# 5l1v3r1/PBS

Measured on AMD Instinct MI355X. Metric: co-run slowdown (%) vs solo + aggregate throughput, 4-tenant mix at 1/2/4/8 GPU, higher is better.
Workload: dtype bf16

## Files before the change

csrc/hip/common.hpp:

```cpp
#pragma once
#include <hip/hip_runtime.h>

#include <cstdint>
#include <cstdio>
#include <cstdlib>

namespace gpbs_hip {

constexpr int kXcds = 8;
constexpr int kMaxTenants = 64;
constexpr int kNumPmc = 4;
constexpr uint32_t kNoOwner = 0xFFFFFFFFu;
constexpr uint32_t kSplitBit = 0x80000000u;
constexpr uint32_t kOwnerMask = 0x7FFFFFFFu;

typedef __bf16 bf16x8 __attribute__((ext_vector_type(8)));
typedef float f32x4 __attribute__((ext_vector_type(4)));
typedef float f32x16 __attribute__((ext_vector_type(16)));
typedef unsigned int u32x4 __attribute__((ext_vector_type(4)));
typedef unsigned int u32x2 __attribute__((ext_vector_type(2)));
typedef unsigned short u16;
typedef unsigned int u32;
typedef unsigned long long u64;

constexpr int kCtx = 4;
struct alignas(64) PartTable {
  u32 epoch;
  u32 flags;
  u32 hold;
  u32 pad0;
  union {
    u32 owner[kXcds * kCtx];
    u64 pair[kXcds][2];
  };
  u32 pad[12];
};
static_assert(sizeof(PartTable) == 192, "partition table layout");

struct alignas(64) WorkQueue {
  u32 next;
  u32 done;
  u32 exited;
  u32 stopped;
  u32 xnext[kXcds];
  u32 pad[4];
};

__device__ __forceinline__ void finish(WorkQueue* q, u32* status, u32 total) {
  if (threadIdx.x == 0) {
    asm volatile("s_waitcnt vmcnt(0)" ::: "memory");
    const u32 old = atomicAdd(&q->exited, 1u);
    if (old == gridDim.x - 1) {
      const u32 d = __hip_atomic_load(&q->done, __ATOMIC_RELAXED, __HIP_MEMORY_SCOPE_AGENT);
      if (status) __hip_atomic_store(status, d | 0x80000000u, __ATOMIC_RELAXED, __HIP_MEMORY_SCOPE_SYSTEM);
      __hip_atomic_store(&q->exited, 0u, __ATOMIC_RELAXED, __HIP_MEMORY_SCOPE_AGENT);
      __hip_atomic_store(&q->stopped, 0u, __ATOMIC_RELAXED, __HIP_MEMORY_SCOPE_AGENT);
      if (d >= total) {
        __hip_atomic_store(&q->next, 0u, __ATOMIC_RELAXED, __HIP_MEMORY_SCOPE_AGENT);
        __hip_atomic_store(&q->done, 0u, __ATOMIC_RELAXED, __HIP_MEMORY_SCOPE_AGENT);
#pragma unroll
        for (int x = 0; x < kXcds; ++x) __hip_atomic_store(&q->xnext[x], 0u, __ATOMIC_RELAXED, __HIP_MEMORY_SCOPE_AGENT);
      }
    }
  }
}


enum GateMode : u32 {
  GATE_NONE = 0, GATE_TABLE = 1, GATE_PARK = 2, GATE_DEVTABLE = 4, GATE_SPATIAL = 8,
  GATE_WAVEPRIO = 16,
  GATE_SE = 32,
  GATE_HOLD = 64,
};
constexpr u32 kParkSpins = 100;
constexpr u32 kHoldSpins = 256;

#define HIPCHECK(x)                                                                              \
  do {                                                                                           \
    hipError_t _e = (x);                                                                         \
    if (_e != hipSuccess) {                                                                      \
      fprintf(stderr, "[gpbs-hip] %s:%d %s -> %s\n", __FILE__, __LINE__, #x, hipGetErrorString(_e)); \
      return -(int)_e - 1000;                                                                    \
    }                                                                                            \
  } while (0)

__device__ __forceinline__ u32 xcc_id() {
  return __builtin_amdgcn_s_getreg((3 << 11) | (0 << 6) | 20);
}

__device__ __forceinline__ u32 hw_id() { return __builtin_amdgcn_s_getreg((31 << 11) | (0 << 6) | 4); }

__device__ __forceinline__ u32 cu_half() { return (hw_id() >> 14) & 1u; }

__device__ __forceinline__ u32 se_id() { return (hw_id() >> 13) & 3u; }

__device__ __forceinline__ u32 load_sys(const u32* p) {
  return __hip_atomic_load(p, __ATOMIC_RELAXED, __HIP_MEMORY_SCOPE_SYSTEM);
}

__device__ __forceinline__ void hold_wait(const PartTable* t, u32 mode) {
  if (!(mode & GATE_HOLD)) return;
  for (u32 k = 0; k < kHoldSpins; ++k) {
    const u32 h = (mode & GATE_DEVTABLE) ? __hip_atomic_load(&t->hold, __ATOMIC_RELAXED, __HIP_MEMORY_SCOPE_AGENT)
                                         : __hip_atomic_load(&t->hold, __ATOMIC_RELAXED, __HIP_MEMORY_SCOPE_SYSTEM);
    if (!h) return;
    __builtin_amdgcn_s_sleep(32);
  }
}

__device__ __forceinline__ bool owns(const PartTable* t, u32 mode, u32 me, u32 xcc) {
  if ((mode & 3) == GATE_NONE) return true;
  if (mode & GATE_SE) {
    const u32 se = se_id();
    const u32* w = t->owner + kCtx * (xcc & 7) + se;
    const u32 o = (mode & GATE_DEVTABLE) ? __hip_atomic_load(w, __ATOMIC_RELAXED, __HIP_MEMORY_SCOPE_AGENT)
                                         : __hip_atomic_load(w, __ATOMIC_RELAXED, __HIP_MEMORY_SCOPE_SYSTEM);
    return (o & kOwnerMask) == me;
  }
  const u64* q = t->pair[xcc & 7];
  const u64 p01 = (mode & GATE_DEVTABLE) ? __hip_atomic_load(q, __ATOMIC_RELAXED, __HIP_MEMORY_SCOPE_AGENT)
                                         : __hip_atomic_load(q, __ATOMIC_RELAXED, __HIP_MEMORY_SCOPE_SYSTEM);
  const u32 w0 = (u32)p01, w1 = (u32)(p01 >> 32);
  const bool h0 = (w0 & kOwnerMask) == me, h1 = (w1 & kOwnerMask) == me;
  if (!(mode & GATE_SPATIAL) || (h0 && h1)) {
    if (h0 || h1) return true;
    const u64 p23 = (mode & GATE_DEVTABLE) ? __hip_atomic_load(q + 1, __ATOMIC_RELAXED, __HIP_MEMORY_SCOPE_AGENT)
                                           : __hip_atomic_load(q + 1, __ATOMIC_RELAXED, __HIP_MEMORY_SCOPE_SYSTEM);
    return (u32)p23 == me || (u32)(p23 >> 32) == me;
  }
  if (h0) return !(w0 & kSplitBit) || cu_half() == 0;
  if (h1) return !(w1 & kSplitBit) || cu_half() == 1;
  return false;
}

__device__ __forceinline__ void count(u64* cnt, u32 me, u32 xcc, u64 inst, u64 cyc, u64 refs, u64 miss) {
  if (!cnt) return;
  u64* c = cnt + ((size_t)me * kXcds + (xcc & 7)) * kNumPmc;
  if (inst) __hip_atomic_fetch_add(c + 0, inst, __ATOMIC_RELAXED, __HIP_MEMORY_SCOPE_SYSTEM);
  if (cyc) __hip_atomic_fetch_add(c + 1, cyc, __ATOMIC_RELAXED, __HIP_MEMORY_SCOPE_SYSTEM);
  if (refs) __hip_atomic_fetch_add(c + 2, refs, __ATOMIC_RELAXED, __HIP_MEMORY_SCOPE_SYSTEM);
  if (miss) __hip_atomic_fetch_add(c + 3, miss, __ATOMIC_RELAXED, __HIP_MEMORY_SCOPE_SYSTEM);
}

__device__ __forceinline__ int grab_unit(WorkQueue* q, const PartTable* table, u32 mode, u32 me, u32 xcc,
                                         int* s_slot, u32 total) {
  if (threadIdx.x == 0) {
    int u = -1;
    hold_wait(table, mode);
    for (u32 spins = 0;; ++spins) {
      if (owns(table, mode, me, xcc)) {
        const u32 t = atomicAdd(&q->next, 1u);
        u = t < total ? (int)t : -1;
        break;
      }
      if ((mode & 3) != GATE_PARK || spins >= kParkSpins ||
          __hip_atomic_load(&q->next, __ATOMIC_RELAXED, __HIP_MEMORY_SCOPE_AGENT) >= total) {
        atomicAdd(&q->stopped, 1u);
        break;
      }
#pragma unroll
      for (int k = 0; k < 6; ++k) __builtin_amdgcn_s_sleep(127);
    }
    *s_slot = u;
  }
  __syncthreads();
  int u = *s_slot;
  __syncthreads();
  return u;
}


__device__ __forceinline__ void count_unit(u64* cnt, u32 me, u32 xcc, u64 inst, u64* t_last, u64 refs, u64 miss,
                                           WorkQueue* q) {
  if (threadIdx.x != 0) return;
  const u64 t = __builtin_amdgcn_s_memtime();
  count(cnt, me, xcc, inst, t - *t_last, refs, miss);
  *t_last = t;
  atomicAdd(&q->done, 1u);
}

}
```

csrc/hip/tenant_kernels.hip:

```cpp
#include "common.hpp"

namespace gpbs_hip {


__device__ __forceinline__ int grab_unit_x(WorkQueue* q, const PartTable* table, u32 mode, u32 me, u32 xcc,
                                           int* s_slot, u32 total) {
  if (threadIdx.x == 0) {
    int u = -1;
    hold_wait(table, mode);
    const u32 per = (total + kXcds - 1) / kXcds;
    for (u32 spins = 0;; ++spins) {
      if (owns(table, mode, me, xcc)) {
        for (u32 k = 0; k < (u32)kXcds; ++k) {
          const u32 r = (xcc + k) & (kXcds - 1);
          const u32 lo = r * per, hi = min(lo + per, total);
          if (lo >= hi) continue;
          if (__hip_atomic_load(&q->xnext[r], __ATOMIC_RELAXED, __HIP_MEMORY_SCOPE_AGENT) >= hi - lo) continue;
          const u32 t = atomicAdd(&q->xnext[r], 1u);
          if (t < hi - lo) {
            u = (int)(lo + t);
            atomicAdd(&q->next, 1u);
            break;
          }
        }
        break;
      }
      if ((mode & 3) != GATE_PARK || spins >= kParkSpins ||
          __hip_atomic_load(&q->next, __ATOMIC_RELAXED, __HIP_MEMORY_SCOPE_AGENT) >= total) {
        atomicAdd(&q->stopped, 1u);
        break;
      }
#pragma unroll
      for (int k = 0; k < 6; ++k) __builtin_amdgcn_s_sleep(127);
    }
    *s_slot = u;
  }
  __syncthreads();
  int u = *s_slot;
  __syncthreads();
  return u;
}


__device__ __forceinline__ u16 f2bf(float x) { return __builtin_bit_cast(u16, (__bf16)x); }
__device__ __forceinline__ float bf2f(u16 x) { return __uint_as_float(((u32)x) << 16); }

constexpr int GBM = 128, GBN = 128, GBK = 64, GNT = 256;
constexpr int kGemmLds = 2 * 2 * GBM * GBK * 2;

typedef __attribute__((address_space(3))) char lds_t;

__device__ __forceinline__ void glds16(const void* g, lds_t* l) {
  __builtin_amdgcn_global_load_lds(g, (__attribute__((address_space(3))) void*)l, 16, 0, 0);
}

__global__ __launch_bounds__(GNT, 2) void k_gemm_bf16_tn(const u16* __restrict__ A, const u16* __restrict__ Bt,
                                                         u16* __restrict__ C, int M, int N, int K, WorkQueue* q,
                                                         const PartTable* table, u32 mode, u32 me, u64* cnt,
                                                         u32 inst_per_tile, u32 refs_per_tile, u32 miss_per_tile,
                                                         u32* status) {
  __shared__ __attribute__((aligned(16))) char smem[kGemmLds + 16];
  lds_t* lds = (lds_t*)smem;
  int* s_slot = (int*)(smem + kGemmLds);
  const u32 xcc = xcc_id();
  u64 t_last = __builtin_amdgcn_s_memtime();
  const int tid = threadIdx.x, lane = tid & 63, wid = tid >> 6;
  const int wr = wid >> 1, wc = wid & 1;
  const int tiles_m = M / GBM, tiles_n = N / GBN, ntiles = tiles_m * tiles_n;
  const int nk = K / GBK;
  constexpr int GROUP_M = 8;

  int srow[4], scol[4];
#pragma unroll
  for (int j = 0; j < 4; ++j) {
    const int c = wid * 4 + j;
    srow[j] = 8 * c + (lane >> 3);
    scol[j] = (((lane & 7) ^ (srow[j] & 7)) * 8);
  }

  for (;;) {
    const int t = grab_unit(q, table, mode, me, xcc, s_slot, (u32)ntiles);
    if (t < 0) break;
    const int in_group = GROUP_M * tiles_n;
    const int g = t / in_group;
    const int first_m = g * GROUP_M;
    const int gsz = min(tiles_m - first_m, GROUP_M);
    const int tm = first_m + (t % in_group) % gsz;
    const int tn = (t % in_group) / gsz;
    const u16* Ab = A + (size_t)tm * GBM * K;
    const u16* Bb = Bt + (size_t)tn * GBN * K;

    f32x4 acc[4][4];
#pragma unroll
// ... 5 lines not shown
      lds_t* la = lds + buf * (2 * GBM * GBK * 2);
      lds_t* lb = la + GBM * GBK * 2;
#pragma unroll
      for (int j = 0; j < 4; ++j) {
        const int c = wid * 4 + j;
        glds16(Ab + (size_t)srow[j] * K + kt * GBK + scol[j], la + c * 1024);
        glds16(Bb + (size_t)srow[j] * K + kt * GBK + scol[j], lb + c * 1024);
      }
    };

    stage(0, 0);
    asm volatile("s_waitcnt vmcnt(0)" ::: "memory");
    __syncthreads();
    int cur = 0;
    for (int kt = 0; kt < nk; ++kt) {
      if (kt + 1 < nk) stage(cur ^ 1, kt + 1);
      const lds_t* la = lds + cur * (2 * GBM * GBK * 2);
      const lds_t* lb = la + GBM * GBK * 2;
#pragma unroll
      for (int s = 0; s < 2; ++s) {
        bf16x8 a[4], b[4];
        const int chunk = s * 4 + (lane >> 4);
#pragma unroll
        for (int i = 0; i < 4; ++i) {
          const int ra = wr * 64 + i * 16 + (lane & 15);
          a[i] = *(const __attribute__((address_space(3))) bf16x8*)(la + ra * 128 + ((chunk ^ (ra & 7)) << 4));
          const int rb = wc * 64 + i * 16 + (lane & 15);
          b[i] = *(const __attribute__((address_space(3))) bf16x8*)(lb + rb * 128 + ((chunk ^ (rb & 7)) << 4));
        }
#pragma unroll
        for (int i = 0; i < 4; ++i)
#pragma unroll
          for (int j = 0; j < 4; ++j) acc[i][j] = __builtin_amdgcn_mfma_f32_16x16x32_bf16(a[i], b[j], acc[i][j], 0, 0, 0);
      }
      asm volatile("s_waitcnt vmcnt(0)" ::: "memory");
      __syncthreads();
      cur ^= 1;
    }
#pragma unroll
    for (int i = 0; i < 4; ++i)
#pragma unroll
      for (int j = 0; j < 4; ++j) {
        const int m = tm * GBM + wr * 64 + i * 16 + (lane >> 4) * 4;
        const int n = tn * GBN + wc * 64 + j * 16 + (lane & 15);
#pragma unroll
        for (int r = 0; r < 4; ++r) C[(size_t)(m + r) * N + n] = f2bf(acc[i][j][r]);
      }
    count_unit(cnt, me, xcc, inst_per_tile, &t_last, refs_per_tile, miss_per_tile, q);
  }
  finish(q, status, (u32)ntiles);
}

constexpr int G2_BM = 256, G2_BK = 64, G2_NT = 512;
constexpr u32 kGemmXRange = 1u << 16;
constexpr u32 kGemmBlock2D = 1u << 17;
constexpr u32 kGemmStatic = 1u << 18;
constexpr int kGemmOptsLive = 1 | 8 | 1 << 23;
constexpr int kGemmOptsShipped = 256 | 8192 | 65536 | 131072;
static int g_gemm_opts = 8;
constexpr int kG2Half = 128 * 128;
constexpr int kG2Buf = 4 * kG2Half;
constexpr int kG2Lds = 2 * kG2Buf;

__device__ __forceinline__ int g2_swz(int r) { return (r >> 1) & 7; }

__global__ __launch_bounds__(G2_NT, 1) void k_gemm256_bf16_tn(const u16* __restrict__ A, const u16* __restrict__ Bt,
                                                             u16* __restrict__ C, int M, int N, int K, WorkQueue* q,
                                                             const PartTable* table, u32 mode, u32 me, u64* cnt,
                                                             u32 inst_per_tile, u32 refs_per_tile, u32 miss_per_tile,
                                                             u32* status) {
  __shared__ __attribute__((aligned(16))) char smem[kG2Lds + 16];
  lds_t* lds = (lds_t*)smem;
  int* s_slot = (int*)(smem + kG2Lds);
  const u32 xcc = xcc_id();
  u64 t_last = __builtin_amdgcn_s_memtime();
  const int tid = threadIdx.x, lane = tid & 63, wid = tid >> 6;
  const int wu = __builtin_amdgcn_readfirstlane(wid);
  const int wr = wu >> 2, wc = wu & 3;
  const int tiles_m = M / G2_BM, tiles_n = N / G2_BM, ntiles = tiles_m * tiles_n;
  const int nt = K / G2_BK;
  int soff[2];
#pragma unroll
  for (int j = 0; j < 2; ++j) {
    const int row = 8 * (2 * wid + j) + (lane >> 3);
    soff[j] = row * K + (((lane & 7) ^ g2_swz(row)) * 8);
  }
  int soffa[4];
#pragma unroll
  for (int j = 0; j < 4; ++j) {
    const int row = 8 * (4 * (wid & 3) + j) + (lane >> 3);
    soffa[j] = row * K + (((lane & 7) ^ g2_swz(row)) * 8);
  }
  const int l16 = lane & 15, lq = lane >> 4;
  const int bh = wc >> 1, bc = (wc & 1) * 64;
  int units_seen = 0;

  for (;;) {
    const int tile = (mode & kGemmStatic) ? (units_seen ? -1 : (int)blockIdx.x)
                     : (mode & kGemmXRange) ? grab_unit_x(q, table, mode, me, xcc, s_slot, (u32)ntiles)
                                            : grab_unit(q, table, mode, me, xcc, s_slot, (u32)ntiles);
    if (tile < 0) break;
    int tm = tile / tiles_n, tn = tile % tiles_n;
    if ((mode & kGemmBlock2D) && (tiles_m & 3) == 0 && (tiles_n & 1) == 0 && ntiles % kXcds == 0) {
      const int per = ntiles / kXcds;
      const int bm = tiles_m / 4, bn = tiles_n / 2;
      const int g = (mode & kGemmXRange) ? tile / per : tile % kXcds;
      const int jj = (mode & kGemmXRange) ? tile % per : tile / kXcds;
      tm = (g >> 1) * bm + jj / bn;
      tn = (g & 1) * bn + jj % bn;
    }
    const u16* Ab = A + (size_t)tm * G2_BM * K;
    const u16* Bb = Bt + (size_t)tn * G2_BM * K;
    auto stage = [&](int kind, int h, int t) {
      const u16* src = (kind ? Bb : Ab) + (size_t)h * 128 * K + t * G2_BK;
      lds_t* dst = lds + (t & 1) * kG2Buf + (kind * 2 + h) * kG2Half + wid * 2048;
      glds16(src + soff[0], dst);
      glds16(src + soff[1], dst + 1024);
    };
    auto stage_own_a = [&](int t) {
      const u16* src = Ab + (size_t)wr * 128 * K + t * G2_BK;
      lds_t* dst = lds + (t & 1) * kG2Buf + wr * kG2Half + (wid & 3) * 4096;
#pragma unroll
      for (int j = 0; j < 4; ++j) glds16(src + soffa[j], dst + j * 1024);
    };
    auto frag = [&](int b, int kind, int h, int r0, int s) -> bf16x8 {
      const int r = r0 + l16;
      const lds_t* p = lds + b * kG2Buf + (kind * 2 + h) * kG2Half + r * 128 + (((4 * s + lq) ^ g2_swz(r)) << 4);
      return *(const __attribute__((address_space(3))) bf16x8*)p;
    };
    f32x4 acc[8][4];
#pragma unroll
    for (int i = 0; i < 8; ++i)
#pragma unroll
      for (int j = 0; j < 4; ++j) acc[i][j] = f32x4{0.f, 0.f, 0.f, 0.f};
    stage(1, 0, 0); stage(1, 1, 0); stage(0, 0, 0); stage(0, 1, 0);
    asm volatile("s_waitcnt vmcnt(0)" ::: "memory");
    __builtin_amdgcn_s_barrier();
    if (wr == 1) __builtin_amdgcn_s_barrier();
    bf16x8 a[4][2], b[4][2];
    for (int t = 0; t < nt; ++t) {
      const int buf = t & 1;
      const bool more = t + 1 < nt;
#pragma unroll
      for (int j = 0; j < 4; ++j)
#pragma unroll
        for (int s2 = 0; s2 < 2; ++s2) b[j][s2] = frag(buf, 1, bh, bc + j * 16, s2);
      __builtin_amdgcn_sched_barrier(0);
#pragma unroll
      for (int i = 0; i < 4; ++i)
#pragma unroll
        for (int s2 = 0; s2 < 2; ++s2) a[i][s2] = frag(buf, 0, wr, i * 16, s2);
      if (more) {
        stage(1, 0, t + 1); stage(1, 1, t + 1);
      } else {
        asm volatile("s_waitcnt vmcnt(0)" ::: "memory");
      }
      __builtin_amdgcn_s_barrier();
      asm volatile("s_waitcnt lgkmcnt(0)" ::: "memory");
      __builtin_amdgcn_s_setprio(1);
#pragma unroll
      for (int s2 = 0; s2 < 2; ++s2)
#pragma unroll
        for (int i = 0; i < 4; ++i)
// ... 41 lines not shown
      const int row = p * 16 + (tid >> 5), c16 = tid & 31;
      u32x4 v = *(const __attribute__((address_space(3))) u32x4*)(lds + row * 512 + (((2 * c16) ^ (row & 14)) << 3));
      if (row & 1) v = u32x4{v.z, v.w, v.x, v.y};
      u32x4* dst = (u32x4*)(C + (size_t)(tm * G2_BM + row) * N + tn * G2_BM + c16 * 8);
      __builtin_nontemporal_store(v, dst);
    }
    __syncthreads();
    ++units_seen;
    if (!(mode & kGemmStatic)) count_unit(cnt, me, xcc, inst_per_tile, &t_last, refs_per_tile, miss_per_tile, q);
  }
  if (!(mode & kGemmStatic)) finish(q, status, (u32)ntiles);
}

constexpr int SNT = 256, SUNROLL = 16, RUNROLL = 6;

template <int U, bool NTS>
__global__ __launch_bounds__(SNT) void k_stream_copy(const f32x4* __restrict__ src, f32x4* __restrict__ dst,
                                                    u64 n4, u32 chunk4, WorkQueue* q, const PartTable* table, u32 mode,
                                                    u32 me, u64* cnt, u32* status) {
  __shared__ int s_slot[4];
  const u32 xcc = xcc_id();
  u64 t_last = __builtin_amdgcn_s_memtime();
  const u32 nchunks = (u32)((n4 + chunk4 - 1) / chunk4);
  const u64 lines = (u64)chunk4 * 16 / 128;
  const u64 inst = (u64)chunk4 * 2 / 64 + 8;
  for (;;) {
    const int c = grab_unit(q, table, mode, me, xcc, s_slot, nchunks);
    if (c < 0) break;
    const u64 base = (u64)c * chunk4;
    const u64 end = min(base + chunk4, n4);
    for (u64 i = base + threadIdx.x; i < end; i += (u64)SNT * U) {
      f32x4 v[U];
#pragma unroll
      for (int k = 0; k < U; ++k) {
        const u64 idx = i + (u64)k * SNT;
        if (idx < end) v[k] = __builtin_nontemporal_load(src + idx);
      }
#pragma unroll
      for (int k = 0; k < U; ++k) {
        const u64 idx = i + (u64)k * SNT;
        if (idx < end) {
          if constexpr (NTS)
            __builtin_nontemporal_store(v[k], dst + idx);
          else
            dst[idx] = v[k];
        }
      }
    }
    count_unit(cnt, me, xcc, inst, &t_last, 2 * lines, 2 * lines, q);
  }
  finish(q, status, nchunks);
}

template <int NT, int U, bool NTL, bool NTS>
__global__ __launch_bounds__(NT) void k_reduce_bf16(const u32x4* __restrict__ a, const u32x4* __restrict__ b,
                                                    u32x4* __restrict__ out, u64 n8, u32 chunk8, WorkQueue* q,
                                                    const PartTable* table, u32 mode, u32 me, u64* cnt,
                                                    u32* status) {
  __shared__ int s_slot[4];
  const u32 xcc = xcc_id();
  u64 t_last = __builtin_amdgcn_s_memtime();
  const u32 nchunks = (u32)((n8 + chunk8 - 1) / chunk8);
  const u64 lines = (u64)chunk8 * 16 / 128;
  const u64 inst = (u64)chunk8 * 3 / 64 + (u64)chunk8 * 16 / 64;
  for (;;) {
    const int c = grab_unit(q, table, mode, me, xcc, s_slot, nchunks);
    if (c < 0) break;
    const u64 base = (u64)c * chunk8, end = min(base + chunk8, n8);
    for (u64 i = base + threadIdx.x; i < end; i += (u64)NT * U) {
      u32x4 x[U], y[U];
#pragma unroll
      for (int k = 0; k < U; ++k) {
        const u64 idx = i + (u64)k * NT;
        if (idx < end) {
          if constexpr (NTL) {
            x[k] = __builtin_nontemporal_load(a + idx);
            y[k] = __builtin_nontemporal_load(b + idx);
          } else {
            x[k] = a[idx];
            y[k] = b[idx];
          }
        }
      }
#pragma unroll
      for (int k = 0; k < U; ++k) {
        const u64 idx = i + (u64)k * NT;
        if (idx >= end) continue;
        const u32* px = (const u32*)&x[k];
        const u32* py = (const u32*)&y[k];
        u32x4 r;
        u32* pr = (u32*)&r;
#pragma unroll
        for (int w = 0; w < 4; ++w) {
          const float lo = bf2f((u16)(px[w] & 0xffff)) + bf2f((u16)(py[w] & 0xffff));
          const float hi = bf2f((u16)(px[w] >> 16)) + bf2f((u16)(py[w] >> 16));
          pr[w] = (u32)f2bf(lo) | ((u32)f2bf(hi) << 16);
        }
        if constexpr (NTS)
          __builtin_nontemporal_store(r, out + idx);
        else
          out[idx] = r;
      }
    }
    count_unit(cnt, me, xcc, inst, &t_last, 3 * lines, 3 * lines, q);
  }
  finish(q, status, nchunks);
}

// ... 65 lines not shown

__global__ void k_census(u32* out, const PartTable* table, u32 mode, u32 me) {
  const u32 xcc = xcc_id();
  const bool ok = owns(table, mode, me, xcc);
  if (threadIdx.x == 0) {
    out[blockIdx.x * 4 + 0] = xcc;
    out[blockIdx.x * 4 + 1] = hw_id();
    out[blockIdx.x * 4 + 2] = ok ? 1u : 0u;
    out[blockIdx.x * 4 + 3] = 0xC0FFEEu;
  }
  if (ok) {
    u64 t = __builtin_amdgcn_s_memtime();
    while (__builtin_amdgcn_s_memtime() - t < 2000) __builtin_amdgcn_s_sleep(1);
  }
}

}

using namespace gpbs_hip;

extern "C" {

int gpbs_hip_set_gemm_opts(int opts) {
  const int old = g_gemm_opts;
  if (opts < 0) return old;
  const int gone = opts & ~(kGemmOptsLive | kGemmOptsShipped);
  static bool warned = false;
  if (gone && !warned) {
    warned = true;
    fprintf(stderr,
            "gpbs_hip_set_gemm_opts: bits 0x%x select GEMM variants that were removed (docs/gemm_lab.md); "
            "the shipped schedule runs\n",
            gone);
  }
  g_gemm_opts = opts & kGemmOptsLive;
  return old;
}

int gpbs_hip_gemm_units(int M, int N) {
  if (M % G2_BM == 0 && N % G2_BM == 0) return (M / G2_BM) * (N / G2_BM);
  return (M / GBM) * (N / GBN);
}

int gpbs_hip_gemm_bf16(const void* A, const void* Bt, void* C, int M, int N, int K, void* q, const void* table,
                       unsigned mode, unsigned me, void* cnt, void* status, int grid, hipStream_t s) {
  if (M % GBM || N % GBN || K % GBK || M <= 0 || N <= 0 || K <= 0) return -22;
  if (M % G2_BM == 0 && N % G2_BM == 0) {
    const int ntiles = (M / G2_BM) * (N / G2_BM);
    if (grid <= 0) grid = 256;
    if (grid > ntiles) grid = ntiles;
    const u32 inst = (u32)((G2_BM / 16) * (G2_BM / 16) * (K / 32) + (K / G2_BK) * 64 + 128);
    const u32 refs = (u32)(((u64)2 * G2_BM * K * 2) / 128);
    const u32 miss = (u32)((((u64)M + N) * K * 2 / 128) / ntiles + (u64)G2_BM * G2_BM * 2 / 128);
    const u32 m2 = mode | ((g_gemm_opts & 1) ? kGemmXRange : 0u) |
                   ((g_gemm_opts & 8) && ntiles % kXcds == 0 ? kGemmBlock2D : 0u) |
                   ((g_gemm_opts & (1 << 23)) && (mode & 3) == GATE_NONE && grid == ntiles ? kGemmStatic : 0u);
    hipLaunchKernelGGL(k_gemm256_bf16_tn, dim3(grid), dim3(G2_NT), 0, s, (const u16*)A, (const u16*)Bt, (u16*)C, M, N,
                       K, (WorkQueue*)q, (const PartTable*)table, m2, me, (u64*)cnt, inst, refs, miss, (u32*)status);
    return hipGetLastError() == hipSuccess ? 0 : -5;
  }
  const int ntiles = (M / GBM) * (N / GBN);
  if (grid <= 0) grid = 256 * 2;
  if (grid > ntiles) grid = ntiles;
  const u32 inst = (u32)((GBM / 16) * (GBN / 16) * (K / 32) * 2 + (K / GBK) * 32 + 64);
  const u32 refs = (u32)(((u64)(GBM + GBN) * K * 2) / 128);
  const u32 miss = (u32)((((u64)M + N) * K * 2 / 128) / ntiles + (u64)GBM * GBN * 2 / 128);
  hipLaunchKernelGGL(k_gemm_bf16_tn, dim3(grid), dim3(GNT), 0, s, (const u16*)A, (const u16*)Bt, (u16*)C, M, N, K,
                     (WorkQueue*)q, (const PartTable*)table, mode, me, (u64*)cnt, inst, refs, miss, (u32*)status);
  return hipGetLastError() == hipSuccess ? 0 : -5;
}

static int g_stream_opts = 0;

int gpbs_hip_set_stream_opts(int opts) {
  const int old = g_stream_opts;
  if (opts >= 0) g_stream_opts = opts;
  return old;
}

int gpbs_hip_stream_copy(const void* src, void* dst, unsigned long long bytes, unsigned chunk_bytes, void* q,
                         const void* table, unsigned mode, unsigned me, void* cnt, void* status, int grid, hipStream_t s) {
  if (bytes % 16 || chunk_bytes % 16 || chunk_bytes == 0) return -22;
  if (grid <= 0) grid = 256;
  using K = void (*)(const f32x4*, f32x4*, u64, u32, WorkQueue*, const PartTable*, u32, u32, u64*, u32*);
  static const K tab[4] = {k_stream_copy<SUNROLL, true>, k_stream_copy<SUNROLL, false>, k_stream_copy<8, true>,
                           k_stream_copy<8, false>};
  hipLaunchKernelGGL(tab[g_stream_opts & 3], dim3(grid), dim3(SNT), 0, s, (const f32x4*)src, (f32x4*)dst, bytes / 16,
                     chunk_bytes / 16, (WorkQueue*)q, (const PartTable*)table, mode, me, (u64*)cnt, (u32*)status);
  return hipGetLastError() == hipSuccess ? 0 : -5;
}

static int g_reduce_opts = 8;

int gpbs_hip_set_reduce_opts(int opts) {
  const int old = g_reduce_opts;
  if (opts >= 0) g_reduce_opts = opts;
  return old;
}

int gpbs_hip_reduce_bf16(const void* a, const void* b, void* out, unsigned long long bytes, unsigned chunk_bytes,
                         void* q, const void* table, unsigned mode, unsigned me, void* cnt, void* status, int grid, hipStream_t s) {
  if (bytes % 16 || chunk_bytes % 16 || chunk_bytes == 0) return -22;
  if (grid <= 0) grid = 256;
  using K = void (*)(const u32x4*, const u32x4*, u32x4*, u64, u32, WorkQueue*, const PartTable*, u32, u32, u64*, u32*);
#define RV(NT, U) {k_reduce_bf16<NT, U, true, true>, k_reduce_bf16<NT, U, false, true>, \
                   k_reduce_bf16<NT, U, true, false>, k_reduce_bf16<NT, U, false, false>}
  static const K table256[4][4] = {RV(256, 6), RV(256, 8), RV(256, 4), RV(256, 12)};
  static const K table512[4][4] = {RV(512, 6), RV(512, 8), RV(512, 4), RV(512, 12)};
#undef RV
  const int o = g_reduce_opts;
  const int nt = (o & 16) ? 512 : 256;
  const K kern = ((o & 16) ? table512 : table256)[o & 3][((o >> 2) & 1) | (((o >> 3) & 1) << 1)];
  hipLaunchKernelGGL(kern, dim3(grid), dim3(nt), 0, s, (const u32x4*)a, (const u32x4*)b, (u32x4*)out,
                     bytes / 16, chunk_bytes / 16, (WorkQueue*)q, (const PartTable*)table, mode, me, (u64*)cnt, (u32*)status);
  return hipGetLastError() == hipSuccess ? 0 : -5;
}

int gpbs_hip_gemv_bf16(const void* W, const void* x, void* y, int R, int K, void* q, const void* table, unsigned mode,
                       unsigned me, void* cnt, void* status, int grid, hipStream_t s) {
  if (K % 512 || R <= 0) return -22;
  if (grid <= 0) grid = (R + 15) / 16;
  if (grid > 256) grid = 256;
  hipLaunchKernelGGL(k_gemv_bf16, dim3(grid), dim3(256), 0, s, (const u16*)W, (const u16*)x, (float*)y, R, K,
                     (WorkQueue*)q, (const PartTable*)table, mode, me, (u64*)cnt, (u32*)status);
  return hipGetLastError() == hipSuccess ? 0 : -5;
}

int gpbs_hip_census(void* out, int blocks, const void* table, unsigned mode, unsigned me, hipStream_t s) {
  hipLaunchKernelGGL(k_census, dim3(blocks), dim3(64), 0, s, (u32*)out, (const PartTable*)table, mode, me);
  return hipGetLastError() == hipSuccess ? 0 : -5;
}

}
```

csrc/hip/runtime.cpp:

```cpp
#include <hip/hip_runtime.h>
#include <hsa/hsa.h>
#include <hsa/hsa_ext_amd.h>
#include <rocprofiler-sdk-roctx/roctx.h>
#include <x86intrin.h>

#include <algorithm>
#include <atomic>
#include <cmath>
#include <cstdio>
#include <cstdlib>
#include <chrono>
#include <condition_variable>
#include <cstring>
#include <deque>
#include <memory>
#include <mutex>
#include <thread>
#include <vector>

#include "../include/gpbs/gpbs.h"
#include "common.hpp"
#include "hwc_attr.h"

using namespace gpbs_hip;
// ... 1414 lines not shown
        hipEventDestroy(retired_ev[i]);
        retired_ev[i] = retired_ev.back();
        retired_ev.pop_back();
      } else {
        ++i;
      }
    hipEvent_t e = nullptr;
    if (hipEventCreateWithFlags(&e, hipEventDisableTiming) != hipSuccess) {
      hipStreamSynchronize(s);
      return;
    }
    hipEventRecord(e, s);
    retired_ev.push_back(e);
  }
  void drain_retired() {
    for (hipEvent_t e : retired_ev) {
      hipEventSynchronize(e);
      hipEventDestroy(e);
    }
    retired_ev.clear();
  }
  uint32_t key_bits = 0;
  int key_half = -1;
  double key_load = 0;
  int64_t rate_t0 = 0;
  uint64_t rate_l0 = 0;
  int cur_grid = 0;
  WorkQueue* d_q = nullptr;
  u32* h_status = nullptr;
  int nq = 0;
  std::thread th;
  std::mutex mu;
  std::condition_variable cv, idle_cv;
  int64_t pending = 0;
  int64_t inflight = 0;
  bool stop = false;
  std::deque<int64_t> submit_times;
  gpbs_runner_stats_t st{};
  std::vector<int64_t> lats;
  hipEvent_t ev[16];
  int err = 0;
  uint64_t q_hold[16] = {};

  void hold_drop(int qi) {
    if (q_hold[qi]) {
      hold_release(ctx, q_hold[qi] - 1);
      q_hold[qi] = 0;
    }
  }

  std::atomic<int> phase{0};
  uint8_t q_alt[16] = {};
  int cur_alt = 0;
  u32 q_seq[16] = {};
  u32 coll_seq = 0;
  int64_t q_t0[16] = {};

  struct Work {
    int kind, M, N, K, chunk;
    unsigned long long bytes;
    void *a, *b, *c;
  };
  static int coll_timeout_ms(const Work& w) { return w.K > 0 ? w.K : 5000; }
  Work work(int alt) const {
    if (alt && cfg.alt_kind)
      return Work{cfg.alt_kind, cfg.alt_M, cfg.alt_N, cfg.alt_K, cfg.alt_chunk_bytes, cfg.alt_bytes,
                  cfg.alt_a, cfg.alt_b, cfg.alt_c};
    return Work{cfg.kind, cfg.M, cfg.N, cfg.K, cfg.chunk_bytes, cfg.bytes, cfg.a, cfg.b, cfg.c};
  }

  static u32 unit_total(const Work& w) {
    switch (w.kind) {
      case K_ALLREDUCE: {
        const u64 n8 = w.bytes / 16, chunk8 = (u64)w.chunk / 16, per = (n8 + w.M - 1) / w.M;
        const u64 lo = (u64)w.N * per, hi = std::min(lo + per, n8);
        return hi > lo ? (u32)((hi - lo + chunk8 - 1) / chunk8) : 0u;
      }
      case K_GEMM: return (u32)gpbs_hip_gemm_units(w.M, w.N);
      case K_GEMM_FP8: return (u32)gpbs_hip_gemm_fp8_units(w.M, w.N);
      case K_STREAM:
      case K_REDUCE: return (u32)((w.bytes + w.chunk - 1) / w.chunk);
      case K_GEMV: return (u32)((w.M + 15) / 16);
    }
    return 0;
  }

  hipStream_t pick_se_stream() {
    u32 any = 0, bits = 0;
    for (int x = 0; x < kXcds; ++x)
      for (int e = 0; e < kCtx; ++e)
        if ((__atomic_load_n(&ctx->h_table->owner[kCtx * x + e], __ATOMIC_ACQUIRE) & kOwnerMask) == (u32)cfg.tenant) {
          any |= 1u << e;
          bits |= 1u << (kCtx * x + e);
        }
    const int half = (any & ~0x3u) == 0 ? 0 : ((any & ~0xCu) == 0 ? 1 : -1);
    if (!any || half < 0) return stream;
    if (!key_stream || bits != key_bits || half != key_half) {
      uint32_t m[8];
      se_half_mask(half, m);
      if (key_stream) {
        retire_stream(key_stream);
        masked_pool().release(key_stream, key_load);
      }
      const int64_t tnow = mono_ns();
      key_load = rate_t0 && tnow > rate_t0 ? (double)(st.launches - rate_l0) * 1e9 / (double)(tnow - rate_t0) : 0.0;
      rate_t0 = tnow;
// ... 24 lines not shown
        se_stream[half ^ 1] = nullptr;
      }
      se_half_mask(half, m);
      se_stream[half] = masked_acquire(m);
      if (!se_stream[half]) return stream;
    }
    return se_stream[half];
  }

  hipStream_t pick_stream() {
    cur_grid = 0;
    const bool se = __atomic_load_n(&ctx->se_mode, __ATOMIC_ACQUIRE);
    const int lh = __atomic_load_n(&ctx->lat_half, __ATOMIC_ACQUIRE);
    if (cfg.priority > 0 && !cfg.gate && lh >= 0) return half_se_stream(lh & 1);
    if (shared()) return stream;
    if (cfg.gate && se) return pick_se_stream();
    if (!ctx->spatial || !cfg.gate) return stream;
    int half = -1;
    for (int x = 0; x < kXcds; ++x) {
      const u32 w0 = __atomic_load_n(&ctx->h_table->owner[kCtx * x], __ATOMIC_ACQUIRE);
      const u32 w1 = __atomic_load_n(&ctx->h_table->owner[kCtx * x + 1], __ATOMIC_ACQUIRE);
      const bool h0 = (w0 & kOwnerMask) == (u32)cfg.tenant, h1 = (w1 & kOwnerMask) == (u32)cfg.tenant;
      if (!h0 && !h1) continue;
      if ((h0 && h1) || !(w0 & kSplitBit)) return stream;
      const int k = h0 ? 0 : 1;
      if (half >= 0 && half != k) return stream;
      half = k;
    }
    if (half < 0) return stream;
    const int k = half;
    if (!half_stream[k]) half_stream[k] = make_half_stream(k);
    return half_stream[k] ? half_stream[k] : stream;
  }

  int launch(int qi, hipStream_t stream) {
    WorkQueue* q = d_q + qi;
    const Work w = work(q_alt[qi]);
    const int tm = __atomic_load_n(&ctx->table_mode, __ATOMIC_ACQUIRE);
    const bool dev = tm != 0;
    const void* tab = tm == 1 ? (const void*)ctx->d_table : tm == 2 ? (const void*)ctx->b_table : (const void*)ctx->h_table;
    const bool gate = cfg.gate && !ctx->share.load(std::memory_order_acquire);
    const bool hold = gate && ctx->hold_enable && tm != 1 && w.kind != K_GEMV && ctx->engine &&
                      ctx->cls_cache[cfg.tenant].load(std::memory_order_relaxed) == 1;
    const unsigned mode = (gate ? (cfg.gate == 2 ? GATE_PARK : GATE_TABLE) : GATE_NONE) | (dev ? GATE_DEVTABLE : 0) |
                          (gate && ctx->spatial ? GATE_SPATIAL : 0) |
                          (gate && __atomic_load_n(&ctx->se_mode, __ATOMIC_ACQUIRE) ? GATE_SE : 0) |
                          (cfg.priority > 0 && ctx->waveprio ? GATE_WAVEPRIO : 0) | (hold ? GATE_HOLD : 0);
    const unsigned me = (unsigned)cfg.tenant;
    __atomic_store_n(&h_status[qi], 0u, __ATOMIC_RELEASE);
    st.launches++;
    const int grid = cfg.grid ? cfg.grid : cur_grid;
    switch (w.kind) {
      case K_GEMM:
        return gpbs_hip_gemm_bf16(w.a, w.b, w.c, w.M, w.N, w.K, q, tab, mode, me, ctx->d_cnt, &h_status[qi], grid,
                                  stream);
      case K_GEMM_FP8: {
        const char *aq = (const char*)w.a, *bq = (const char*)w.b;
        return gpbs_hip_gemm_fp8(aq, (const float*)(aq + (size_t)w.M * w.K), bq, (const float*)(bq + (size_t)w.N * w.K),
                                 w.c, w.M, w.N, w.K, 0, q, tab, mode, me, ctx->d_cnt, &h_status[qi], grid, stream);
      }
      case K_STREAM:
        return gpbs_hip_stream_copy(w.a, w.c, w.bytes, (unsigned)w.chunk, q, tab, mode, me, ctx->d_cnt,
                                    &h_status[qi], grid, stream);
      case K_REDUCE:
        return gpbs_hip_reduce_bf16(w.a, w.b, w.c, w.bytes, (unsigned)w.chunk, q, tab, mode, me, ctx->d_cnt,
                                    &h_status[qi], grid, stream);
      case K_GEMV:
        return gpbs_hip_gemv_bf16(w.a, w.b, w.c, w.M, w.K, q, tab, mode, me, ctx->d_cnt, &h_status[qi], grid,
                                  stream);
      case K_ALLREDUCE:
        return gpbs_hip_allreduce(w.a, q_seq[qi], w.bytes, (unsigned)w.chunk, q, tab, mode, me, ctx->d_cnt,
                                  &h_status[qi], grid, (unsigned long long)coll_timeout_ms(w) * 100000ull,
                                  100000ull, stream);
    }
    return -22;
  }

  bool owns_any() {
    if (!cfg.gate || shared()) return true;
    for (int x = 0; x < kXcds * kCtx; ++x)
      if ((__atomic_load_n(&ctx->h_table->owner[x], __ATOMIC_ACQUIRE) & kOwnerMask) == (u32)cfg.tenant) return true;
    return false;
  }

  int wo_qi = -1;
  int64_t q_l0[16] = {};
  int64_t drain_seen_rv = 0;
  int64_t ramp_from = 0;
  static void ewma(std::atomic<int64_t>& a, std::atomic<uint64_t>& n, int64_t v) {
    const int64_t o = a.load(std::memory_order_relaxed);
    a.store(n.load(std::memory_order_relaxed) ? o + (v - o) / 8 : v, std::memory_order_relaxed);
    n.fetch_add(1, std::memory_order_relaxed);
  }
  void note_drain(int qi, int64_t now) {
    if (cfg.tenant < 0 || cfg.tenant >= kMaxTenants) return;
    const int64_t rv = ctx->revoke_ns[cfg.tenant].load(std::memory_order_relaxed);
    if (!rv || rv == drain_seen_rv || rv < q_l0[qi] || now < rv) return;
    const u32 s = __atomic_load_n(&h_status[qi], __ATOMIC_ACQUIRE);
    if ((s & 0x80000000u) && (s & 0x3fffffffu) >= unit_total(work(q_alt[qi]))) return;
    drain_seen_rv = rv;
    const int64_t dr = now - rv;
    if (dr >= 1000000000) return;
    st.drain_sum_ns += dr;
    st.drain_count++;
    if (dr > st.drain_max_ns) st.drain_max_ns = dr;
    ewma(ctx->swc_drain_ns[cfg.tenant], ctx->swc_drain_n[cfg.tenant], dr);
  }
  void note_ramp(int64_t now) {
// ... 31 lines not shown
      gpbs_slot_wake(ctx->engine, cfg.tenant, -1);
    else
      gpbs_slot_block(ctx->engine, cfg.tenant, -1);
  }

  void loop() {
    hipSetDevice(ctx->device);
    struct Fl {
      int qi;
      int ev;
    };
    std::deque<Fl> fl;
    int next_q = 0;
    std::vector<char> q_busy(nq, 0);
    for (;;) {
      {
        std::unique_lock<std::mutex> lk(mu);
        cv.wait(lk, [&] { return stop || pending > 0; });
        if (stop) break;
      }
      engine_wake(true);
      const int64_t batch_t0 = mono_ns();
      if (!st.first_start_ns) st.first_start_ns = batch_t0;
      std::deque<int> relaunch;
      for (;;) {
        for (;;) {
          if ((int)fl.size() >= cfg.depth) break;
          int qi = -1;
          bool fresh = false;
          if (!relaunch.empty()) {
            qi = relaunch.front();
          } else {
            std::lock_guard<std::mutex> g(mu);
            if (pending <= 0) break;
            for (int k = 0; k < nq; ++k) {
              int cand = (next_q + k) % nq;
              if (!q_busy[cand]) {
                qi = cand;
                break;
              }
            }
            if (qi < 0) break;
            fresh = true;
          }
          wo_qi = fl.empty() ? -1 : fl.front().qi;
          wait_owner();
          if (stop) break;
          if (fresh) {
            q_alt[qi] = (uint8_t)(cfg.alt_kind && phase.load(std::memory_order_acquire));
            q_seq[qi] = coll_seq++;
            q_t0[qi] = mono_ns();
          }
          cur_alt = q_alt[qi];
          hipStream_t stream = pick_stream();
          if (fresh) {
            std::lock_guard<std::mutex> g(mu);
            pending--;
            inflight++;
            next_q = (qi + 1) % nq;
            q_busy[qi] = 1;
          } else {
            relaunch.pop_front();
            st.relaunches++;
          }
          if (cfg.priority > 0 && ctx->hold_enable && fresh && !q_hold[qi]) q_hold[qi] = hold_acquire(ctx) + 1;
          q_l0[qi] = mono_ns();
          note_ramp(q_l0[qi]);
          if (launch(qi, stream) != 0) err = -5;
          const int e = qi;
          hipEventRecord(ev[e], stream);
          fl.push_back({qi, e});
        }
        if (fl.empty()) {
          std::lock_guard<std::mutex> g(mu);
          if (pending <= 0 && relaunch.empty()) break;
          continue;
        }
        Fl f = fl.front();
        fl.pop_front();
        while (hipEventQuery(ev[f.ev]) == hipErrorNotReady) {
          if (stop) break;
          std::this_thread::yield();
        }
        const u32 s = __atomic_load_n(&h_status[f.qi], __ATOMIC_ACQUIRE);
        const u32 done = s & 0x3fffffffu;
        const Work fw = work(q_alt[f.qi]);
        const bool unfinished = !((s & 0x80000000u) && done >= unit_total(fw));
        const bool coll_late = fw.kind == K_ALLREDUCE && unfinished &&
                               mono_ns() - q_t0[f.qi] > (int64_t)coll_timeout_ms(fw) * 1000000;
        if (((s & 0x80000000u) && (s & 0x40000000u)) || coll_late) {
          std::fprintf(stderr, "[gpbs-hip] tenant %d: collective unit %u timed out waiting for its peers\n",
                       cfg.tenant, q_seq[f.qi]);
          err = -110;
          hold_drop(f.qi);
          std::lock_guard<std::mutex> g(mu);
          q_busy[f.qi] = 0;
          inflight--;
          pending = 0;
          if (!submit_times.empty()) submit_times.pop_front();
        } else if ((s & 0x80000000u) && done >= unit_total(work(q_alt[f.qi]))) {
          hold_drop(f.qi);
          const int64_t t = mono_ns();
          std::lock_guard<std::mutex> g(mu);
          q_busy[f.qi] = 0;
          inflight--;
          st.units_done++;
// ... 1817 lines not shown
```

Before: 1.267.

## Software-pipeline bf16 reduce with buffer loads and overlapped chunk claiming

Rewrites the bf16 reduce kernel as a software pipeline. Each iteration stores the sum of the previous batch while loading the next batch through buffer resource descriptors with hardware bounds clamping, which removes per-element index checks. The next work unit is claimed inside the walk using a single barrier and double-buffered shared slots, replacing the two syncthreads per grab. The old kernel is kept as a batch variant behind an opts bit. This adds a chunk-size limit and an extra store of zeros on the first iteration, clamped away by the empty descriptor.

```diff
diff --git a/csrc/hip/common.hpp b/csrc/hip/common.hpp
--- a/csrc/hip/common.hpp
+++ b/csrc/hip/common.hpp
@@ -169,6 +169,23 @@
   return u;
 }
 
+__device__ __forceinline__ int claim_unit(WorkQueue* q, const PartTable* table, u32 mode, u32 me, u32 xcc, u32 total) {
+  hold_wait(table, mode);
+  for (u32 spins = 0;; ++spins) {
+    if (owns(table, mode, me, xcc)) {
+      const u32 t = atomicAdd(&q->next, 1u);
+      return t < total ? (int)t : -1;
+    }
+    if ((mode & 3) != GATE_PARK || spins >= kParkSpins ||
+        __hip_atomic_load(&q->next, __ATOMIC_RELAXED, __HIP_MEMORY_SCOPE_AGENT) >= total) {
+      atomicAdd(&q->stopped, 1u);
+      return -1;
+    }
+#pragma unroll
+    for (int k = 0; k < 6; ++k) __builtin_amdgcn_s_sleep(127);
+  }
+}
+
 
 __device__ __forceinline__ void count_unit(u64* cnt, u32 me, u32 xcc, u64 inst, u64* t_last, u64 refs, u64 miss,
                                            WorkQueue* q) {
diff --git a/csrc/hip/tenant_kernels.hip b/csrc/hip/tenant_kernels.hip
--- a/csrc/hip/tenant_kernels.hip
+++ b/csrc/hip/tenant_kernels.hip
@@ -354,8 +354,96 @@
   finish(q, status, nchunks);
 }
 
+constexpr unsigned kMaxChunkBytes = 0xFFF00000u;
+constexpr int kBufNT = 2;
+
+__device__ __forceinline__ __amdgpu_buffer_rsrc_t chunk_rsrc(const void* base, u64 off16, u32 len16) {
+  return __builtin_amdgcn_make_buffer_rsrc((void*)((const char*)base + off16 * 16), 0, (int)(len16 * 16u), 0x00020000);
+}
+
+struct ChunkWalk {
+  u64 sbase, lbase;
+  u32 slen, llen;
+  u32 spos, lpos;
+  bool slast;
+};
+
+__device__ __forceinline__ void walk_start(ChunkWalk& w, int c, u64 n, u32 chunk) {
+  w.sbase = 0, w.slen = 0, w.spos = 0, w.slast = false;
+  w.lbase = (u64)c * chunk, w.llen = (u32)min((u64)chunk, n - w.lbase), w.lpos = 0;
+}
+
+__device__ __forceinline__ bool walk_next(ChunkWalk& w, u32 batch, u64 n, u32 chunk, WorkQueue* q,
+                                          const PartTable* table, u32 mode, u32 me, u32 xcc, u32 nchunks, int* s_slot,
+                                          u32& par) {
+  if (w.llen == 0) return false;
+  w.sbase = w.lbase, w.slen = w.llen, w.spos = w.lpos;
+  w.slast = w.lpos + batch >= w.llen;
+  if (!w.slast) {
+    w.lpos += batch;
+    return true;
+  }
+  if (threadIdx.x == 0) s_slot[par] = claim_unit(q, table, mode, me, xcc, nchunks);
+  asm volatile("s_waitcnt lgkmcnt(0)" ::: "memory");
+  __builtin_amdgcn_s_barrier();
+  asm volatile("" ::: "memory");
+  const int nxt = __builtin_amdgcn_readfirstlane(s_slot[par]);
+  par ^= 1;
+  w.lpos = 0, w.llen = 0;
+  if (nxt >= 0) w.lbase = (u64)nxt * chunk, w.llen = (u32)min((u64)chunk, n - w.lbase);
+  return true;
+}
+
+__device__ __forceinline__ u32x4 add_bf16x8(const u32x4 x, const u32x4 y) {
+  u32x4 r;
+#pragma unroll
+  for (int w = 0; w < 4; ++w) {
+    const float lo = bf2f((u16)(x[w] & 0xffff)) + bf2f((u16)(y[w] & 0xffff));
+    const float hi = bf2f((u16)(x[w] >> 16)) + bf2f((u16)(y[w] >> 16));
+    r[w] = (u32)f2bf(lo) | ((u32)f2bf(hi) << 16);
+  }
+  return r;
+}
+
 template <int NT, int U, bool NTL, bool NTS>
 __global__ __launch_bounds__(NT) void k_reduce_bf16(const u32x4* __restrict__ a, const u32x4* __restrict__ b,
+                                                    u32x4* __restrict__ out, u64 n8, u32 chunk8, WorkQueue* q,
+                                                    const PartTable* table, u32 mode, u32 me, u64* cnt,
+                                                    u32* status) {
+  __shared__ int s_slot[4];
+  const u32 xcc = xcc_id();
+  u64 t_last = __builtin_amdgcn_s_memtime();
+  const u32 nchunks = (u32)((n8 + chunk8 - 1) / chunk8);
+  const u64 lines = (u64)chunk8 * 16 / 128;
+  const u64 inst = (u64)chunk8 * 3 / 64 + (u64)chunk8 * 16 / 64;
+  const int c0 = __builtin_amdgcn_readfirstlane(grab_unit(q, table, mode, me, xcc, s_slot, nchunks));
+  if (c0 >= 0) {
+    u32x4 x[U], y[U];
+#pragma unroll
+    for (int k = 0; k < U; ++k) x[k] = y[k] = u32x4{0, 0, 0, 0};
+    ChunkWalk w;
+    walk_start(w, c0, n8, chunk8);
+    u32 par = 1;
+    do {
+      const __amdgpu_buffer_rsrc_t rs = chunk_rsrc(out, w.sbase, w.slen);
+      const __amdgpu_buffer_rsrc_t ra = chunk_rsrc(a, w.lbase, w.llen), rb = chunk_rsrc(b, w.lbase, w.llen);
+      const u32 so = (w.spos + threadIdx.x) * 16, lo = (w.lpos + threadIdx.x) * 16;
+#pragma unroll
+      for (int k = 0; k < U; ++k) {
+        __builtin_amdgcn_raw_buffer_store_b128(add_bf16x8(x[k], y[k]), rs, so + k * NT * 16, 0, NTS ? kBufNT : 0);
+        __builtin_amdgcn_sched_barrier(0);
+        x[k] = __builtin_amdgcn_raw_buffer_load_b128(ra, lo + k * NT * 16, 0, NTL ? kBufNT : 0);
+        y[k] = __builtin_amdgcn_raw_buffer_load_b128(rb, lo + k * NT * 16, 0, NTL ? kBufNT : 0);
+        __builtin_amdgcn_sched_barrier(0);
+      }
+      if (w.slast) count_unit(cnt, me, xcc, inst, &t_last, 3 * lines, 3 * lines, q);
+    } while (walk_next(w, NT * U, n8, chunk8, q, table, mode, me, xcc, nchunks, s_slot, par));
+  }
+  finish(q, status, nchunks);
+}
+
+template <int NT, int U, bool NTL, bool NTS>
+__global__ __launch_bounds__(NT) void k_reduce_bf16_batch(const u32x4* __restrict__ a, const u32x4* __restrict__ b,
                                                     u32x4* __restrict__ out, u64 n8, u32 chunk8, WorkQueue* q,
                                                     const PartTable* table, u32 mode, u32 me, u64* cnt,
                                                     u32* status) {
@@ -575,7 +663,7 @@
 
 int gpbs_hip_reduce_bf16(const void* a, const void* b, void* out, unsigned long long bytes, unsigned chunk_bytes,
                          void* q, const void* table, unsigned mode, unsigned me, void* cnt, void* status, int grid, hipStream_t s) {
-  if (bytes % 16 || chunk_bytes % 16 || chunk_bytes == 0) return -22;
+  if (bytes % 16 || chunk_bytes % 16 || chunk_bytes == 0 || chunk_bytes > kMaxChunkBytes) return -22;
   if (grid <= 0) grid = 256;
   using K = void (*)(const u32x4*, const u32x4*, u32x4*, u64, u32, WorkQueue*, const PartTable*, u32, u32, u64*, u32*);
 #define RV(NT, U) {k_reduce_bf16<NT, U, true, true>, k_reduce_bf16<NT, U, false, true>, \
@@ -585,7 +673,8 @@
 #undef RV
   const int o = g_reduce_opts;
   const int nt = (o & 16) ? 512 : 256;
-  const K kern = ((o & 16) ? table512 : table256)[o & 3][((o >> 2) & 1) | (((o >> 3) & 1) << 1)];
+  K kern = ((o & 16) ? table512 : table256)[o & 3][((o >> 2) & 1) | (((o >> 3) & 1) << 1)];
+  if ((o & 63) == (8 | 32)) kern = k_reduce_bf16_batch<256, 6, true, false>;
   hipLaunchKernelGGL(kern, dim3(grid), dim3(nt), 0, s, (const u32x4*)a, (const u32x4*)b, (u32x4*)out,
                      bytes / 16, chunk_bytes / 16, (WorkQueue*)q, (const PartTable*)table, mode, me, (u64*)cnt, (u32*)status);
   return hipGetLastError() == hipSuccess ? 0 : -5;
```

Result: no change. 1.260 (median of 2 runs) (-0.6%).

## Deal GEMM tiles per XCD range with strip order and resume-aware dealing

Applied to the files above, without the earlier changes.

Moves the GEMM tile-to-XCD mapping into a shared helper and adds a strip-ordered variant inside each XCD's 2D block, which is meant to improve L2 reuse of A and B panels. XCD-range dealing now turns on by default when blocking applies and the grid is smaller than the tile count. The per-XCD grab first claims from its own range with a single atomic and then steals from other ranges using a snapshot of their counters. Resumed (preempted) launches are flagged so the kernel reuses the dealing mode the earlier partial run used, keeping tile indices consistent. This adds host/kernel flag plumbing, and the stealing path or mode inference could misassign tiles if it is wrong.

```diff
diff --git a/csrc/hip/common.hpp b/csrc/hip/common.hpp
--- a/csrc/hip/common.hpp
+++ b/csrc/hip/common.hpp
@@ -71,6 +71,7 @@
   GATE_WAVEPRIO = 16,
   GATE_SE = 32,
   GATE_HOLD = 64,
+  GATE_RESUME = 128,
 };
 constexpr u32 kParkSpins = 100;
 constexpr u32 kHoldSpins = 256;
diff --git a/csrc/hip/gemm_deal.hpp b/csrc/hip/gemm_deal.hpp
--- /dev/null
+++ b/csrc/hip/gemm_deal.hpp
@@ -0,0 +1,38 @@
+#pragma once
+
+#if defined(__HIPCC__)
+#define GPBS_DEAL_HD __host__ __device__ __forceinline__
+#else
+#define GPBS_DEAL_HD inline
+#endif
+
+namespace gpbs_hip {
+
+constexpr int kDealXcds = 8;
+constexpr unsigned kGemmXRange = 1u << 16;
+constexpr unsigned kGemmBlock2D = 1u << 17;
+constexpr unsigned kGemmStrip = 1u << 19;
+
+struct GemmTile {
+  int tm, tn;
+};
+
+GPBS_DEAL_HD bool gemm_deal_blocks(int tiles_m, int tiles_n) {
+  return (tiles_m & 3) == 0 && (tiles_n & 1) == 0 && (tiles_m * tiles_n) % kDealXcds == 0;
+}
+
+GPBS_DEAL_HD int gemm_deal_per(int ntiles) { return (ntiles + kDealXcds - 1) / kDealXcds; }
+
+GPBS_DEAL_HD GemmTile gemm_deal_tile(int unit, int tiles_m, int tiles_n, unsigned mode) {
+  if (!(mode & kGemmBlock2D) || !gemm_deal_blocks(tiles_m, tiles_n)) return GemmTile{unit / tiles_n, unit % tiles_n};
+  const int per = tiles_m * tiles_n / kDealXcds;
+  const int bm = tiles_m / 4, bn = tiles_n / 2;
+  const bool ranges = (mode & kGemmXRange) != 0;
+  const int g = ranges ? unit / per : unit % kDealXcds;
+  const int jj = ranges ? unit % per : unit / kDealXcds;
+  const int w = (ranges && (mode & kGemmStrip) && !(bn & 1)) ? bn / 2 : bn;
+  const int s = jj / (bm * w), r = jj % (bm * w);
+  return GemmTile{(g >> 1) * bm + r / w, (g & 1) * bn + s * w + r % w};
+}
+
+}
diff --git a/csrc/hip/runtime.cpp b/csrc/hip/runtime.cpp
--- a/csrc/hip/runtime.cpp
+++ b/csrc/hip/runtime.cpp
@@ -1490,6 +1490,7 @@
   std::atomic<int> phase{0};
   uint8_t q_alt[16] = {};
   int cur_alt = 0;
+  bool cur_resume = false;
   u32 q_seq[16] = {};
   u32 coll_seq = 0;
   int64_t q_t0[16] = {};
@@ -1620,8 +1621,8 @@
     const int grid = cfg.grid ? cfg.grid : cur_grid;
     switch (w.kind) {
       case K_GEMM:
-        return gpbs_hip_gemm_bf16(w.a, w.b, w.c, w.M, w.N, w.K, q, tab, mode, me, ctx->d_cnt, &h_status[qi], grid,
-                                  stream);
+        return gpbs_hip_gemm_bf16(w.a, w.b, w.c, w.M, w.N, w.K, q, tab, mode | (cur_resume ? GATE_RESUME : 0u), me,
+                                  ctx->d_cnt, &h_status[qi], grid, stream);
       case K_GEMM_FP8: {
         const char *aq = (const char*)w.a, *bq = (const char*)w.b;
         return gpbs_hip_gemm_fp8(aq, (const float*)(aq + (size_t)w.M * w.K), bq, (const float*)(bq + (size_t)w.N * w.K),
@@ -1759,6 +1760,7 @@
             q_t0[qi] = mono_ns();
           }
           cur_alt = q_alt[qi];
+          cur_resume = !fresh;
           hipStream_t stream = pick_stream();
           if (fresh) {
             std::lock_guard<std::mutex> g(mu);
diff --git a/csrc/hip/tenant_kernels.hip b/csrc/hip/tenant_kernels.hip
--- a/csrc/hip/tenant_kernels.hip
+++ b/csrc/hip/tenant_kernels.hip
@@ -1,4 +1,5 @@
 #include "common.hpp"
+#include "gemm_deal.hpp"
 
 namespace gpbs_hip {
 
@@ -8,21 +9,35 @@
   if (threadIdx.x == 0) {
     int u = -1;
     hold_wait(table, mode);
-    const u32 per = (total + kXcds - 1) / kXcds;
+    const u32 per = (u32)gemm_deal_per((int)total);
+    auto size_of = [&](u32 r) { return r * per < total ? min(per, total - r * per) : 0u; };
     for (u32 spins = 0;; ++spins) {
       if (owns(table, mode, me, xcc)) {
-        for (u32 k = 0; k < (u32)kXcds; ++k) {
-          const u32 r = (xcc + k) & (kXcds - 1);
-          const u32 lo = r * per, hi = min(lo + per, total);
-          if (lo >= hi) continue;
-          if (__hip_atomic_load(&q->xnext[r], __ATOMIC_RELAXED, __HIP_MEMORY_SCOPE_AGENT) >= hi - lo) continue;
-          const u32 t = atomicAdd(&q->xnext[r], 1u);
-          if (t < hi - lo) {
-            u = (int)(lo + t);
-            atomicAdd(&q->next, 1u);
-            break;
+        const u32 x = xcc & (kXcds - 1);
+        const u32 own = size_of(x);
+        const u32 t = own ? (u32)__builtin_amdgcn_readfirstlane(atomicAdd(&q->xnext[x], 1u)) : 0u;
+        if (t < own) {
+          u = (int)(x * per + t);
+        } else {
+          u32 seen[kXcds];
+#pragma unroll
+          for (int r = 0; r < kXcds; ++r)
+            seen[r] = __hip_atomic_load(&q->xnext[r], __ATOMIC_RELAXED, __HIP_MEMORY_SCOPE_AGENT);
+          for (u32 k = 1; k < (u32)kXcds; ++k) {
+            const u32 r = (x + k) & (kXcds - 1);
+            u32 sr = 0;
+#pragma unroll
+            for (int i = 0; i < kXcds; ++i) sr = (u32)i == r ? seen[i] : sr;
+            const u32 sz = size_of(r);
+            if ((u32)__builtin_amdgcn_readfirstlane(sr) >= sz) continue;
+            const u32 tr = __builtin_amdgcn_readfirstlane(atomicAdd(&q->xnext[r], 1u));
+            if (tr < sz) {
+              u = (int)(r * per + tr);
+              break;
+            }
           }
         }
+        if (u >= 0) atomicAdd(&q->next, 1u);
         break;
       }
       if ((mode & 3) != GATE_PARK || spins >= kParkSpins ||
@@ -39,6 +54,20 @@
   int u = *s_slot;
   __syncthreads();
   return u;
+}
+
+__device__ __forceinline__ u32 resumed_deal(WorkQueue* q, u32 mode, int* s_slot) {
+  if (threadIdx.x == 0) {
+    const u32 n = __hip_atomic_load(&q->next, __ATOMIC_ACQUIRE, __HIP_MEMORY_SCOPE_AGENT);
+    u32 any = 0;
+#pragma unroll
+    for (int r = 0; r < kXcds; ++r) any |= __hip_atomic_load(&q->xnext[r], __ATOMIC_RELAXED, __HIP_MEMORY_SCOPE_AGENT);
+    *s_slot = (int)(any ? (mode | kGemmXRange) : n ? (mode & ~kGemmXRange) : mode);
+  }
+  __syncthreads();
+  const u32 m = (u32)*s_slot;
+  __syncthreads();
+  return __builtin_amdgcn_readfirstlane(m);
 }
 
 
@@ -150,10 +179,8 @@
 }
 
 constexpr int G2_BM = 256, G2_BK = 64, G2_NT = 512;
-constexpr u32 kGemmXRange = 1u << 16;
-constexpr u32 kGemmBlock2D = 1u << 17;
 constexpr u32 kGemmStatic = 1u << 18;
-constexpr int kGemmOptsLive = 1 | 8 | 1 << 23;
+constexpr int kGemmOptsLive = 1 | 8 | 1 << 23 | 1 << 24 | 1 << 25;
 constexpr int kGemmOptsShipped = 256 | 8192 | 65536 | 131072;
 static int g_gemm_opts = 8;
 constexpr int kG2Half = 128 * 128;
@@ -192,21 +219,15 @@
   const int l16 = lane & 15, lq = lane >> 4;
   const int bh = wc >> 1, bc = (wc & 1) * 64;
   int units_seen = 0;
+  if (mode & GATE_RESUME) mode = resumed_deal(q, mode, s_slot);
 
   for (;;) {
     const int tile = (mode & kGemmStatic) ? (units_seen ? -1 : (int)blockIdx.x)
                      : (mode & kGemmXRange) ? grab_unit_x(q, table, mode, me, xcc, s_slot, (u32)ntiles)
                                             : grab_unit(q, table, mode, me, xcc, s_slot, (u32)ntiles);
     if (tile < 0) break;
-    int tm = tile / tiles_n, tn = tile % tiles_n;
-    if ((mode & kGemmBlock2D) && (tiles_m & 3) == 0 && (tiles_n & 1) == 0 && ntiles % kXcds == 0) {
-      const int per = ntiles / kXcds;
-      const int bm = tiles_m / 4, bn = tiles_n / 2;
-      const int g = (mode & kGemmXRange) ? tile / per : tile % kXcds;
-      const int jj = (mode & kGemmXRange) ? tile % per : tile / kXcds;
-      tm = (g >> 1) * bm + jj / bn;
-      tn = (g & 1) * bn + jj % bn;
-    }
+    const GemmTile tl = gemm_deal_tile(__builtin_amdgcn_readfirstlane(tile), tiles_m, tiles_n, mode);
+    const int tm = tl.tm, tn = tl.tn;
     const u16* Ab = A + (size_t)tm * G2_BM * K;
     const u16* Bb = Bt + (size_t)tn * G2_BM * K;
     auto stage = [&](int kind, int h, int t) {
@@ -527,9 +548,12 @@
     const u32 inst = (u32)((G2_BM / 16) * (G2_BM / 16) * (K / 32) + (K / G2_BK) * 64 + 128);
     const u32 refs = (u32)(((u64)2 * G2_BM * K * 2) / 128);
     const u32 miss = (u32)((((u64)M + N) * K * 2 / 128) / ntiles + (u64)G2_BM * G2_BM * 2 / 128);
-    const u32 m2 = mode | ((g_gemm_opts & 1) ? kGemmXRange : 0u) |
-                   ((g_gemm_opts & 8) && ntiles % kXcds == 0 ? kGemmBlock2D : 0u) |
-                   ((g_gemm_opts & (1 << 23)) && (mode & 3) == GATE_NONE && grid == ntiles ? kGemmStatic : 0u);
+    const bool blocks = (g_gemm_opts & 8) && gemm_deal_blocks(M / G2_BM, N / G2_BM);
+    const bool ranges = (g_gemm_opts & 1) || (blocks && grid < ntiles && !(g_gemm_opts & (1 << 24)));
+    const u32 m2 = mode | (ranges ? kGemmXRange : 0u) | ((g_gemm_opts & 8) && ntiles % kXcds == 0 ? kGemmBlock2D : 0u) |
+                   ((ranges || (mode & GATE_RESUME)) && !(g_gemm_opts & (1 << 25)) ? kGemmStrip : 0u) |
+                   ((g_gemm_opts & (1 << 23)) && (mode & (3 | GATE_RESUME)) == GATE_NONE && grid == ntiles ? kGemmStatic
+                                                                                                         : 0u);
     hipLaunchKernelGGL(k_gemm256_bf16_tn, dim3(grid), dim3(G2_NT), 0, s, (const u16*)A, (const u16*)Bt, (u16*)C, M, N,
                        K, (WorkQueue*)q, (const PartTable*)table, m2, me, (u64*)cnt, inst, refs, miss, (u32*)status);
     return hipGetLastError() == hipSuccess ? 0 : -5;
```

Result: no change. 1.251 before, 1.256 after (median of 5 runs) (+0.4%).
